# tuannv-github/srsRAN_Project

Hardware: AMD Instinct MI355X
Metric: PDSCH+PUSCH codeblocks/s @ 100 MHz 273-PRB 4x4 MIMO (PDSCH 4 layers, PUSCH 4 layers x 4 rx) (higher is better)
Workload: dtype int8+fp32; 1 GPU; BASELINE metric (PDSCH+PUSCH codeblocks/s @ 100 MHz 273-PRB 4x4 MIMO): full PDSCH+PUSCH slot pipeline, 100 MHz numerology-1 273 PRB, 256QAM R=948/1024; parallelism=single GPU

## Files before the change

### srsran_project_amd/csrc/crc_device.h

```cpp
#pragma once

#include <hip/hip_runtime.h>

#include <cstdint>

namespace srs_amd {

__device__ __forceinline__ uint32_t crc_wave_xor(uint32_t v)
{
#pragma unroll
  for (int o = 32; o >= 1; o >>= 1) {
    v ^= static_cast<uint32_t>(__shfl_xor(static_cast<int>(v), o, 64));
  }
  return v;
}

template <int THREADS>
__device__ __forceinline__ void crc_table8_init(uint32_t* T, uint32_t order, uint32_t polynom)
{
  if (order < 8) {
    return;
  }
  const uint32_t highbit = 1u << order;
  for (uint32_t t = threadIdx.x; t < 256; t += THREADS) {
    uint32_t r = t << (order - 8);
#pragma unroll
    for (int i = 0; i < 8; ++i) {
      r <<= 1;
      if (r & highbit) {
        r ^= polynom;
      }
    }
    T[t] = r;
  }
}

constexpr uint32_t CRC_FETCH_BATCH = 16;
constexpr uint32_t CRC_MAX_ORDER = 24;

template <typename Fetch>
__device__ __forceinline__ uint32_t crc_chunk_contrib(const Fetch&    fetch,
                                                      uint32_t        b0,
                                                      uint32_t        b1,
                                                      uint32_t        n,
                                                      uint32_t        order,
                                                      uint32_t        polynom,
                                                      const uint32_t* table,
                                                      const uint32_t* T,
                                                      uint32_t        to = 0xffffffffu)
{
  to = to == 0xffffffffu ? n : to;
  if (b0 >= b1) {
    return 0;
  }
  const uint32_t highbit = 1u << order;
  const uint32_t mask    = highbit - 1u;
  const uint32_t full    = min(b1, n / 8);
  uint32_t       r       = 0;
  uint32_t       b       = b0;
  if (order >= 8) {
    const uint32_t sh = order - 8;
    for (; b < full; b += CRC_FETCH_BATCH) {
      uint32_t v[CRC_FETCH_BATCH];
#pragma unroll
      for (uint32_t k = 0; k < CRC_FETCH_BATCH; ++k) {
        v[k] = b + k < full ? fetch(b + k) : 0u;
      }
#pragma unroll
      for (uint32_t k = 0; k < CRC_FETCH_BATCH; ++k) {
        if (b + k < full) {
          r = T[r >> sh] ^ ((r << 8) & mask) ^ v[k];
        }
      }
    }
    b = max(b0, full);
  }
  for (; b < b1; ++b) {
    const uint32_t byte = fetch(b);
    const int      nb   = (b * 8 + 8 <= n) ? 8 : static_cast<int>(n - b * 8);
    for (int i = 0; i < nb; ++i) {
      r = (r << 1) | ((byte >> (7 - i)) & 1u);
      if (r & highbit) {
        r ^= polynom;
      }
    }
  }
  const uint32_t  e       = min(n, b1 * 8);
  const uint32_t* tj      = table + (to - e);
  uint32_t        contrib = 0;
#pragma unroll
  for (uint32_t j = 0; j < CRC_MAX_ORDER; ++j) {
    if (j < order) {
      contrib ^= tj[j] & (0u - ((r >> j) & 1u));
    }
  }
  return contrib;
}

__device__ __forceinline__ uint32_t crc_move(uint32_t R, uint32_t d, uint32_t order, const uint32_t* table)
{
  uint32_t out = 0;
#pragma unroll
  for (uint32_t j = 0; j < CRC_MAX_ORDER; ++j) {
    const uint32_t k    = j + d;
    const uint32_t word = k >= order ? table[k - order] : 0u;
    const uint32_t v    = k < order ? (1u << (k & 31u)) : word;
    out ^= (j < order) ? (v & (0u - ((R >> j) & 1u))) : 0u;
  }
  return out;
}

template <typename Fetch>
__device__ __forceinline__ uint32_t crc_chunk_rem(const Fetch& fetch, uint32_t b0, uint32_t b1, uint32_t order,
                                                  const uint32_t* T)
{
  const uint32_t mask = (1u << order) - 1u;
  const uint32_t sh   = order - 8;
  uint32_t       r    = 0;
  for (uint32_t b = b0; b < b1; b += CRC_FETCH_BATCH) {
    uint32_t v[CRC_FETCH_BATCH];
#pragma unroll
    for (uint32_t k = 0; k < CRC_FETCH_BATCH; ++k) {
      v[k] = b + k < b1 ? fetch(b + k) : 0u;
    }
#pragma unroll
    for (uint32_t k = 0; k < CRC_FETCH_BATCH; ++k) {
      if (b + k < b1) {
        r = T[r >> sh] ^ ((r << 8) & mask) ^ v[k];
      }
    }
  }
  return r;
}

__device__ __forceinline__ uint32_t crc_mulmod(uint32_t a, uint32_t c, uint32_t order, uint32_t polynom)
{
  const uint32_t mask = (1u << order) - 1u;
  const uint32_t top  = 1u << (order - 1);
  uint32_t       r    = 0;
#pragma unroll
  for (uint32_t i = 0; i < CRC_MAX_ORDER; ++i) {
    if (i < order) {
      r ^= c & (0u - ((a >> i) & 1u));
      const uint32_t hi = c & top;
      c                 = ((c << 1) & mask) ^ (hi ? (polynom & mask) : 0u);
    }
  }
  return r;
}

__device__ __forceinline__ uint32_t crc_xpow(uint32_t m, uint32_t order, const uint32_t* table)
{
  return m < order ? (1u << m) : table[m - order];
}

template <int THREADS>
__device__ __forceinline__ uint32_t crc_block_xor(uint32_t v, uint32_t* partial)
{
  v = crc_wave_xor(v);
  __syncthreads();
  if ((threadIdx.x & 63) == 0) {
    partial[threadIdx.x >> 6] = v;
  }
  __syncthreads();
  uint32_t crc = 0;
#pragma unroll
  for (int w = 0; w < THREADS / 64; ++w) {
    crc ^= partial[w];
  }
  return crc;
}

template <int THREADS, typename Fetch>
__device__ uint32_t block_crc_bytes(const Fetch&    fetch,
                                    uint32_t        n,
                                    uint32_t        order,
                                    uint32_t        polynom,
                                    const uint32_t* table,
                                    const uint32_t* T,
                                    uint32_t*       partial)
{
  const uint32_t nbytes = (n + 7) / 8;
  const uint32_t per    = (nbytes + THREADS - 1) / THREADS;
  const uint32_t b0     = threadIdx.x * per;
  const uint32_t b1     = min(nbytes, b0 + per);
  return crc_block_xor<THREADS>(crc_chunk_contrib(fetch, b0, b1, n, order, polynom, table, T), partial);
}

__device__ __forceinline__ void attach_crc_bits(uint8_t* row, uint32_t n, uint32_t order, uint32_t crc)
{
  const uint32_t first = n >> 3, last = (n + order - 1) >> 3;
  uint32_t       bytes[4];
#pragma unroll
  for (uint32_t k = 0; k < 4; ++k) {
    bytes[k] = first + k <= last ? row[first + k] : 0u;
  }
#pragma unroll
  for (uint32_t k = 0; k < 4; ++k) {
    if (first + k <= last) {
      uint32_t byte = bytes[k];
#pragma unroll
      for (uint32_t b = 0; b < 8; ++b) {
        const uint32_t pos = 8 * (first + k) + b;
        if (pos >= n && pos < n + order) {
          const uint32_t mask = 0x80u >> b;
          byte                = (byte & ~mask) | (((crc >> (order - 1 - (pos - n))) & 1u) ? mask : 0u);
        }
      }
      row[first + k] = static_cast<uint8_t>(byte);
    }
  }
}

template <int THREADS>
__device__ __forceinline__ void crc_stage_bytes(uint8_t* dst, const uint8_t* row, uint32_t c0, uint32_t n)
{
  const uint8_t* src = row + c0;
  uint32_t       nw  = (reinterpret_cast<uintptr_t>(src) & 3u) == 0 ? n / 4 : 0;
  constexpr int  U   = 8;
  for (uint32_t w0 = threadIdx.x; w0 < nw; w0 += U * THREADS) {
    uint32_t v[U];
#pragma unroll
    for (int r = 0; r < U; ++r) {
      const uint32_t w = w0 + r * THREADS;
      v[r]             = w < nw ? reinterpret_cast<const uint32_t*>(src)[w] : 0u;
    }
#pragma unroll
    for (int r = 0; r < U; ++r) {
      const uint32_t w = w0 + r * THREADS;
      if (w < nw) {
        reinterpret_cast<uint32_t*>(dst)[w] = v[r];
      }
    }
  }
  for (uint32_t i = 4 * nw + threadIdx.x; i < n; i += THREADS) {
    dst[i] = src[i];
  }
}

struct row_fetch {
  const uint8_t* row;
  __device__ uint32_t operator()(uint32_t j) const { return row[j]; }
};

struct lds_chunk_fetch {
  const uint8_t* chunk;
  uint32_t       first;
  __device__ uint32_t operator()(uint32_t j) const { return chunk[j - first]; }
};

}
```

### srsran_project_amd/csrc/ldpc_encode_device.h

```cpp
#pragma once

#include <hip/hip_runtime.h>

#include <cstdint>

namespace srs_amd {

__device__ __forceinline__ uint32_t lds_bits32(const uint32_t* W, uint32_t off)
{
  const uint32_t w = off >> 5;
  return __builtin_amdgcn_alignbit(W[w + 1], W[w], off & 31u);
}

__device__ __forceinline__ uint32_t cyc32(const uint32_t* W, uint32_t cz, uint32_t Z, uint32_t x0, uint32_t s)
{
  uint32_t pos = x0 + s;
  pos -= pos >= Z ? Z : 0u;
  uint32_t v = lds_bits32(W, cz + pos);
  if (pos + 32 > Z) {
    const uint32_t n1 = Z - pos;
    v = (v & ((1u << n1) - 1u)) | (lds_bits32(W, cz) << n1);
  }
  return v;
}

__device__ __forceinline__ void lds_or_bits(uint32_t* W, uint32_t off, uint32_t v, uint32_t n)
{
  v &= n < 32 ? (1u << n) - 1u : 0xffffffffu;
  const uint32_t w = off >> 5, sh = off & 31u;
  atomicOr(&W[w], v << sh);
  if (sh != 0) {
    atomicOr(&W[w + 1], v >> (32 - sh));
  }
}

__host__ __device__ constexpr uint32_t enc_bits_cw_words(uint32_t K, uint32_t M_eff, uint32_t Z)
{
  return ((K + M_eff) * Z + 31) / 32 + 2;
}
__host__ __device__ constexpr uint32_t enc_bits_lds_words(uint32_t K, uint32_t M_eff, uint32_t Z)
{
  return enc_bits_cw_words(K, M_eff, Z) + 4 * ((Z + 31) / 32) + (Z + 31) / 32 + 2;
}

template <int NT>
__device__ __forceinline__ void encode_bits_parity(uint32_t*       cw,
                                                   uint32_t*       lam,
                                                   uint32_t*       ls,
                                                   const uint32_t* edges,
                                                   const int32_t*  row_start,
                                                   int             bg,
                                                   uint32_t        K,
                                                   uint32_t        Z,
                                                   uint32_t        M_eff,
                                                   int32_t         p0_shift,
                                                   const int32_t (&core_a)[3],
                                                   uint32_t        j)
{
  const uint32_t kz = K * Z;
  const uint32_t nq = (Z + 31) / 32;
  for (uint32_t task = j; task < 4 * nq; task += NT) {
    const uint32_t r = task / nq, x0 = 32 * (task - r * nq);
    uint32_t       acc = 0;
    for (int e = row_start[r]; e < row_start[r + 1]; ++e) {
      const uint32_t ed   = edges[e];
      const uint32_t base = ed & 0xffffu;
      if (base >= kz) {
        break;
      }
      acc ^= cyc32(cw, base, Z, x0, ed >> 16);
    }
    lam[task] = acc;
  }
  __syncthreads();
  for (uint32_t q = j; q < nq; q += NT) {
    const uint32_t n = min(32u, Z - 32 * q);
    const uint32_t v = lam[q] ^ lam[nq + q] ^ lam[2 * nq + q] ^ lam[3 * nq + q];
    ls[q]            = n < 32 ? v & ((1u << n) - 1u) : v;
  }
  __syncthreads();

  const uint32_t sh0 = (Z - static_cast<uint32_t>(p0_shift) % Z) % Z;
  for (uint32_t q = j; q < nq; q += NT) {
    lds_or_bits(cw, kz + 32 * q, cyc32(ls, 0, Z, 32 * q, sh0), min(32u, Z - 32 * q));
  }
  __syncthreads();

  for (uint32_t q = j; q < nq; q += NT) {
    const uint32_t x0 = 32 * q, n = min(32u, Z - x0);
    auto           at = [&](int s) { return cyc32(cw, kz, Z, x0, static_cast<uint32_t>(s)); };
    uint32_t       p1, p2, p3;
    p1 = lam[q] ^ at(core_a[0]);
    if (bg == 1) {
      p2 = lam[nq + q] ^ at(core_a[1]) ^ p1;
      p3 = lam[2 * nq + q] ^ p2;
    } else {
      p2 = lam[nq + q] ^ p1;
      p3 = lam[2 * nq + q] ^ at(core_a[2]) ^ p2;
    }
    lds_or_bits(cw, kz + Z + x0, p1, n);
    lds_or_bits(cw, kz + 2 * Z + x0, p2, n);
    lds_or_bits(cw, kz + 3 * Z + x0, p3, n);
  }
  __syncthreads();

  const uint32_t hz = kz + 4 * Z;
  for (uint32_t task = j; task < (M_eff - 4) * nq; task += NT) {
    const uint32_t rr = task / nq, r = 4 + rr, x0 = 32 * (task - rr * nq);
    uint32_t       acc = 0;
    for (int e = row_start[r]; e < row_start[r + 1]; ++e) {
      const uint32_t ed   = edges[e];
      const uint32_t base = ed & 0xffffu;
      if (base >= hz) {
        break;
      }
      acc ^= cyc32(cw, base, Z, x0, ed >> 16);
    }
    lds_or_bits(cw, (K + r) * Z + x0, acc, min(32u, Z - x0));
  }
  __syncthreads();
}

}
```

### srsran_project_amd/csrc/pdsch_encoder.hip

```cpp
#include <hip/hip_runtime.h>

#include <algorithm>
#include <atomic>
#include <cstdlib>

#include "crc_device.h"
#include "ldpc_codec_args.h"
#include "ldpc_common.h"
#include "ldpc_encode_device.h"
#include "rate_match_device.h"
#include "sch_args.h"

namespace srs_amd {
namespace {

constexpr uint32_t PE_CW_BYTES  = 66 * MAX_LIFTING_SIZE / 8;
constexpr uint32_t PE_ENC_WORDS = enc_bits_lds_words(22, 46, MAX_LIFTING_SIZE);

__device__ __forceinline__ uint32_t pe_out_byte(const uint8_t* s_cw, const rm_geometry& g, const fast_div& divL,
                                                uint32_t off, uint32_t E, uint32_t Kq, uint32_t b)
{
  uint32_t byte = 0;
#pragma unroll
  for (uint32_t k = 0; k < 8; ++k) {
    const uint32_t gbit = 8 * b + k;
    if (gbit < off || gbit >= off + E) {
      continue;
    }
    const uint32_t o = gbit - off;
    uint32_t       i, j;
    if (g.Qm == 6) {
      i = __umulhi(o >> 1, 0xAAAAAAABu) >> 1;
      j = o - 6 * i;
    } else {
      const uint32_t sh = g.Qm == 8 ? 3 : g.Qm == 4 ? 2 : g.Qm == 2 ? 1 : 0;
      i                 = o >> sh;
      j                 = o & (g.Qm - 1);
    }
    uint32_t w = g.rank0 + j * Kq + i;
    if (w >= g.L) {
      w -= g.L;
      if (w >= g.L) {
        divL.div(w, w);
      }
    }
    const uint32_t p = w < g.nof_info ? w : w + g.F;
    byte |= ((s_cw[p >> 3] >> (7 - (p & 7))) & 1u) << (7 - k);
  }
  return byte;
}

struct pe_lds {
  uint32_t T24b[256];
  uint32_t Ttb[256];
  uint32_t lw[PE_ENC_WORDS];
  uint32_t edges[MAX_EDGES];
  __attribute__((aligned(16))) uint8_t s_cw[PE_CW_BYTES + 8];
  uint32_t partial[4];
};

template <int NT>
__device__ __forceinline__ uint32_t pe_xor(uint32_t v, uint32_t* partial)
{
  if constexpr (NT == 64) {
    return crc_wave_xor(v);
  } else {
    return crc_block_xor<NT>(v, partial);
  }
}

template <int NT>
__device__ __forceinline__ void pe_message(const pdsch_fused_args& a, const tb_desc& d, uint32_t r, uint32_t n_data,
                                           uint32_t kz, uint8_t* s_cw, uint32_t j)
{
  const uint8_t* tb  = a.tbs + d.tb_offset;
  const uint32_t ob  = r * d.cb_info_bits;
  const uint32_t nmb = (kz + 7) / 8;
  if ((ob & 7u) == 0) {
    const uintptr_t base  = reinterpret_cast<uintptr_t>(tb) + ob / 8;
    const uint32_t  nfull = n_data / 32;
    for (uint32_t q = j; q < nfull; q += NT) {
      const uintptr_t  addr = base + 4 * q;
      const uint32_t*  p4   = reinterpret_cast<const uint32_t*>(addr & ~uintptr_t(3));
      const uint32_t   sh   = static_cast<uint32_t>(addr & 3u);
      const uint32_t   lo   = p4[0];
      const uint32_t   hi   = sh != 0 ? p4[1] : 0u;
      reinterpret_cast<uint32_t*>(s_cw)[q] = sh != 0 ? __builtin_amdgcn_alignbyte(hi, lo, sh) : lo;
    }
    for (uint32_t q = nfull + j; q < (nmb + 3) / 4; q += NT) {
      uint32_t w = 0;
      for (uint32_t b = 0; b < 4; ++b) {
        const uint32_t jb = 4 * q + b;
        uint32_t       v  = 0;
        for (uint32_t k = 0; k < 8 && 8 * jb + k < n_data; ++k) {
          const uint32_t p = ob + 8 * jb + k;
          v |= ((tb[p >> 3] >> (7 - (p & 7))) & 1u) << (7 - k);
        }
        w |= v << (8 * b);
      }
      reinterpret_cast<uint32_t*>(s_cw)[q] = w;
    }
    return;
  }
  for (uint32_t q = j; q < (nmb + 3) / 4; q += NT) {
    uint32_t w = 0;
#pragma unroll
    for (uint32_t b = 0; b < 4; ++b) {
      const uint32_t jb = 4 * q + b;
      uint32_t       v  = 0;
      if (8 * jb + 8 <= n_data) {
        const uint32_t p  = ob + 8 * jb;
        const uint32_t sh = p & 7u;
        uint32_t       x  = static_cast<uint32_t>(tb[p >> 3]) << 8;
        if (sh != 0) {
          x |= tb[(p >> 3) + 1];
        }
        v = (x >> (8 - sh)) & 0xffu;
      } else if (8 * jb < n_data) {
        for (uint32_t k = 0; k < 8 && 8 * jb + k < n_data; ++k) {
          const uint32_t p = ob + 8 * jb + k;
          v |= ((tb[p >> 3] >> (7 - (p & 7))) & 1u) << (7 - k);
        }
      }
      w |= v << (8 * b);
    }
    reinterpret_cast<uint32_t*>(s_cw)[q] = w;
  }
}

__device__ __forceinline__ void pe_crc24_pair(const uint8_t* s_cw, uint32_t b0, uint32_t b1, uint32_t n,
                                              uint32_t polyA, const uint32_t* tableA, const uint32_t* TA,
                                              uint32_t polyB, const uint32_t* tableB, const uint32_t* TB,
                                              uint32_t& outA, uint32_t& outB)
{
  outA = 0;
  outB = 0;
  if (b0 >= b1) {
    return;
  }
  constexpr uint32_t highbit = 1u << 24, mask = highbit - 1u;
  const uint32_t     full    = min(b1, n / 8);
  uint32_t           rA = 0, rB = 0;
  for (uint32_t b = b0; b < full; b += CRC_FETCH_BATCH) {
    uint32_t v[CRC_FETCH_BATCH];
#pragma unroll
    for (uint32_t k = 0; k < CRC_FETCH_BATCH; ++k) {
      v[k] = b + k < full ? s_cw[b + k] : 0u;
    }
#pragma unroll
    for (uint32_t k = 0; k < CRC_FETCH_BATCH; ++k) {
      if (b + k < full) {
        rA = TA[rA >> 16] ^ ((rA << 8) & mask) ^ v[k];
        rB = TB[rB >> 16] ^ ((rB << 8) & mask) ^ v[k];
      }
    }
  }
  for (uint32_t b = max(b0, full); b < b1; ++b) {
    const uint32_t byte = s_cw[b];
    const int      nb   = (b * 8 + 8 <= n) ? 8 : static_cast<int>(n - b * 8);
    for (int i = 0; i < nb; ++i) {
      const uint32_t bit = (byte >> (7 - i)) & 1u;
      rA                 = (rA << 1) | bit;
      rB                 = (rB << 1) | bit;
      rA ^= (rA & highbit) ? polyA : 0u;
      rB ^= (rB & highbit) ? polyB : 0u;
    }
  }
  const uint32_t  e  = min(n, b1 * 8);
  const uint32_t* ta = tableA + (n - e);
  const uint32_t* tb = tableB + (n - e);
#pragma unroll
  for (uint32_t j = 0; j < 24; ++j) {
    outA ^= ta[j] & (0u - ((rA >> j) & 1u));
    outB ^= tb[j] & (0u - ((rB >> j) & 1u));
  }
}

template <int NT>
__device__ __forceinline__ void pe_finish(const pdsch_fused_args& a, pe_lds& s, uint32_t cb, uint32_t t,
                                          const tb_desc& d, uint32_t j, uint32_t& staged_off, uint32_t& staged_ne)
{
  const rm_geometry  g   = a.geos[a.row_geo[cb]];
  const enc_row_desc er  = a.enc_rows[cb];
  const uint32_t     E   = a.row_E[cb];
  const uint32_t     off = a.row_out[cb];
  const uint32_t     Z   = er.Z;
  const uint32_t     Kb  = g.nof_sys / Z + 2;
  const int          bg  = Kb == 22 ? 1 : 2;
  const uint32_t     kz  = Kb * Z;
  uint8_t*           s_cw = s.s_cw;
  if (d.nof_segments > 1) {
    const uint32_t cbi = d.cb_info_bits;
    const uint32_t nb  = (cbi + 7) / 8;
    const uint32_t per = (nb + NT - 1) / NT;
    const uint32_t b0  = j * per;
    const uint32_t r   = cb - d.row0;
    uint32_t       crc;
    if (r + 1 < d.nof_segments) {
      uint32_t tb_part;
      pe_crc24_pair(s_cw, b0, min(nb, b0 + per), cbi, a.crc24b_poly, a.crc24b_table, s.T24b, a.crc24a_poly,
                    a.crc24a_table, s.Ttb, crc, tb_part);
      crc     = pe_xor<NT>(crc, s.partial);
      tb_part = pe_xor<NT>(tb_part, s.partial);
      if (j == 0) {
        a.tb_parts[static_cast<size_t>(t) * a.part_stride + r] = tb_part;
      }
    } else {
      crc = pe_xor<NT>(crc_chunk_contrib(lds_chunk_fetch{s_cw, 0}, b0, min(nb, b0 + per), cbi, 24, a.crc24b_poly,
                                         a.crc24b_table, s.T24b),
                       s.partial);
    }
    if (j == 0) {
      attach_crc_bits(s_cw, cbi, 24, crc);
    }
    __syncthreads();
  }
  const uint32_t nq  = (Z + 31) / 32;
  const uint32_t ncw = enc_bits_cw_words(Kb, er.M_eff, Z);
  uint32_t*      cwb = s.lw;
  uint32_t*      lam = s.lw + ncw;
  uint32_t*      ls  = lam + 4 * nq;
  const uint32_t nmw = (kz + 31) / 32;
  for (uint32_t w = j; w < ncw; w += NT) {
    uint32_t v = 0;
    if (w < nmw) {
      v = __builtin_bitreverse32(__builtin_bswap32(reinterpret_cast<const uint32_t*>(s_cw)[w]));
      if (32 * w + 32 > kz) {
        v &= (1u << (kz - 32 * w)) - 1u;
      }
    }
    cwb[w] = v;
  }
  for (uint32_t w = j; w < nq + 2; w += NT) {
    ls[w] = 0;
  }
  const uint32_t* ge = a.edges + er.edge_off;
  const uint32_t  ne = static_cast<uint32_t>(a.row_start[bg - 1][er.M_eff]);
  if (er.edge_off != staged_off || ne != staged_ne) {
    for (uint32_t e = j; e < ne; e += NT) {
      s.edges[e] = ge[e];
    }
    staged_off = er.edge_off;
    staged_ne  = ne;
  }
  __syncthreads();
  const int32_t core_a[3] = {static_cast<int32_t>(er.core_a[0]), static_cast<int32_t>(er.core_a[1]),
                             static_cast<int32_t>(er.core_a[2])};
  encode_bits_parity<NT>(cwb, lam, ls, s.edges, a.row_start[bg - 1], bg, Kb, Z, er.M_eff,
                                 static_cast<int32_t>(er.p0_shift), core_a, j);
  const uint32_t nbits = er.pack_bits;
  for (uint32_t m = j; m < (nbits + 31) / 32; m += NT) {
    uint32_t v = lds_bits32(cwb, 2 * Z + 32 * m);
    if (32 * m + 32 > nbits) {
      v &= (1u << (nbits - 32 * m)) - 1u;
    }
    reinterpret_cast<uint32_t*>(s_cw)[m] = __builtin_bswap32(__builtin_bitreverse32(v));
  }
  __syncthreads();
  const fast_div divL(g.L);
  const uint32_t Kq    = E / g.Qm;
  const uint32_t first = (off + 7) / 8;
  const uint32_t whole = (off + E) / 8;
  const uint32_t G        = ((off & 7u) == 0 && g.Qm >= 2) ? Kq / 8 : 0;
  const uint32_t fast_end = first + G * g.Qm;
  for (uint32_t gi = j; gi < G; gi += NT) {
    uint64_t x = 0;
#pragma unroll
    for (uint32_t jj = 0; jj < 8; ++jj) {
      if (jj < g.Qm) {
        uint32_t w = g.rank0 + jj * Kq + 8 * gi;
        if (w >= g.L) {
          w -= g.L;
          if (w >= g.L) {
            divL.div(w, w);
          }
        }
        x |= static_cast<uint64_t>(rm_walk_byte(s_cw, g, w)) << (56 - 8 * jj);
      }
    }
    x            = transpose8x8(x);
    uint64_t acc = 0;
#pragma unroll
    for (uint32_t q = 0; q < 8; ++q) {
      acc = (acc << g.Qm) | ((x >> (64 - 8 * q - g.Qm)) & ((1u << g.Qm) - 1u));
    }
    uint8_t* o = a.cw + first + gi * g.Qm;
    for (uint32_t q = 0; q < g.Qm; ++q) {
      o[q] = static_cast<uint8_t>(acc >> (8 * (g.Qm - 1 - q)));
    }
  }
  for (uint32_t b = fast_end + j; b < whole; b += NT) {
    a.cw[b] = static_cast<uint8_t>(pe_out_byte(s_cw, g, divL, off, E, Kq, b));
  }
  if (j < 2) {
    const bool     last_seg = cb == d.row0 + d.nof_segments - 1;
    const uint32_t b        = j == 0 ? off / 8 : whole;
    const bool partial =
        j == 0 ? (off & 7u) != 0 : ((off + E) & 7u) != 0 && (whole != off / 8 || (off & 7u) == 0);
    if (partial) {
      uint32_t mask = 0;
      for (uint32_t k = 0; k < 8; ++k) {
        const uint32_t gbit = 8 * b + k;
        mask |= (gbit >= off && (gbit < off + E || last_seg)) ? (0x80u >> k) : 0u;
      }
      const uint32_t v  = pe_out_byte(s_cw, g, divL, off, E, Kq, b);
      uint32_t*      w4 = reinterpret_cast<uint32_t*>(a.cw + (b & ~3u));
      const uint32_t sh = 8 * (b & 3u);
      atomicAnd(w4, ~(mask << sh));
      atomicOr(w4, v << sh);
    }
  }
  __syncthreads();
}

template <int NT>
__global__ __launch_bounds__(NT) void pdsch_cb_kernel(pdsch_fused_args a)
{
  __shared__ pe_lds s;
  crc_table8_init<NT>(s.T24b, 24, a.crc24b_poly);
  crc_table8_init<NT>(s.Ttb, 24, a.crc24a_poly);
  uint32_t       tb_table_order = 24;
  uint32_t       staged_off = 0, staged_ne = 0;
  const uint32_t j              = threadIdx.x;

  const uint32_t n = a.last_only == 1 ? a.nof_tbs : a.nof_cbs;
  for (uint32_t k = blockIdx.x; k < n; k += gridDim.x) {
    const uint32_t cb   = a.last_only == 1 ? a.last_rows[k] : k;
    const uint32_t t    = a.row_tb[cb];
    const tb_desc  d    = a.tds[t];
    const uint32_t r    = cb - d.row0;
    const uint32_t C    = d.nof_segments;
    const bool     last = r == C - 1;
    if ((a.last_only == 0) == last) {
      continue;
    }
    const uint32_t L    = d.tb_crc_bits;
    const uint32_t n_data = last ? d.cb_info_bits - L - d.zero_pad : d.cb_info_bits;
    const uint32_t kz     = (a.geos[a.row_geo[cb]].nof_sys / a.enc_rows[cb].Z + 2) * a.enc_rows[cb].Z;
    uint32_t tb_crc = 0;
    if (last) {
      if (tb_table_order != L) {
        crc_table8_init<NT>(s.Ttb, L, L == 16 ? a.crc16_poly : a.crc24a_poly);
        tb_table_order = L;
      }
      for (uint32_t i = j; i + 1 < C; i += NT) {
        tb_crc ^= crc_move(a.tb_parts[static_cast<size_t>(t) * a.part_stride + i],
                           d.tbs_bits - (i + 1) * d.cb_info_bits, 24, a.crc24a_table);
      }
    }
    pe_message<NT>(a, d, r, n_data, kz, s.s_cw, j);
    __syncthreads();
    if (last) {
      const uint32_t nb  = (n_data + 7) / 8;
      const uint32_t per = (nb + NT - 1) / NT;
      const uint32_t b0  = j * per;
      tb_crc ^= crc_chunk_contrib(lds_chunk_fetch{s.s_cw, 0}, b0, min(nb, b0 + per), n_data, L,
                                  L == 16 ? a.crc16_poly : a.crc24a_poly, L == 16 ? a.crc16_table : a.crc24a_table,
                                  s.Ttb);
      tb_crc = pe_xor<NT>(tb_crc, s.partial);
      if (j == 0) {
        attach_crc_bits(s.s_cw, n_data, L, tb_crc);
      }
      __syncthreads();
    }
    pe_finish<NT>(a, s, cb, t, d, j, staged_off, staged_ne);
  }
}

constexpr int PE_MAX_DEVICES = 64;

template <int NT>
uint32_t pe_resident_workgroups()
{
  static std::atomic<uint32_t> known[PE_MAX_DEVICES] = {};
  int                          dev = 0, per_cu = 0, cus = 0;
  if (hipGetDevice(&dev) != hipSuccess || dev < 0 || dev >= PE_MAX_DEVICES) {
    (void)hipGetLastError();
    return 65535u;
  }
  uint32_t n = known[dev].load(std::memory_order_relaxed);
  if (n == 0) {
    if (hipDeviceGetAttribute(&cus, hipDeviceAttributeMultiprocessorCount, dev) != hipSuccess || cus <= 0 ||
        hipOccupancyMaxActiveBlocksPerMultiprocessor(&per_cu, pdsch_cb_kernel<NT>, NT, 0) != hipSuccess ||
        per_cu <= 0) {
      (void)hipGetLastError();
      return 65535u;
    }
    n = static_cast<uint32_t>(per_cu) * static_cast<uint32_t>(cus);
    known[dev].store(n, std::memory_order_relaxed);
  }
  return n;
}

}

hipError_t launch_pdsch_fused(const pdsch_fused_args& a, hipStream_t stream)
{
  if (a.nof_cbs == 0) {
    return hipSuccess;
  }
  const char* wg       = std::getenv("SRSRAN_AMD_PDSCH_WG");
  const char* tail     = std::getenv("SRSRAN_AMD_PDSCH_TAIL_WG");
  const bool  big      = wg != nullptr && wg[0] == '2';
  const bool  big_tail = tail == nullptr || tail[0] == '2';
  const char*    gs  = std::getenv("SRSRAN_AMD_PDSCH_GRID");
  const uint32_t cap = gs != nullptr && std::atoi(gs) > 0 ? static_cast<uint32_t>(std::atoi(gs))
                       : big                              ? pe_resident_workgroups<256>()
                                                          : pe_resident_workgroups<64>();
  auto cb_launch = [&](uint32_t last_only, uint32_t n, bool wide) {
    pdsch_fused_args x = a;
    x.last_only        = last_only;
    const dim3 grid(std::min(n, last_only == 0 ? std::min(cap, 65535u) : 65535u));
    if (wide) {
      hipLaunchKernelGGL(pdsch_cb_kernel<256>, grid, dim3(256), 0, stream, x);
    } else {
      hipLaunchKernelGGL(pdsch_cb_kernel<64>, grid, dim3(64), 0, stream, x);
    }
  };
  if (a.nof_cbs > a.nof_tbs) {
    cb_launch(0, a.nof_cbs, big);
  }
  cb_launch(1, a.nof_tbs, big_tail);
  return hipGetLastError();
}

}
```

Measured before the change: 25.14 million codeblocks/s.

## Prefetch next codeblock metadata and message, vectorize CRC, group rate matching

The PDSCH fused kernel is restructured so each workgroup prefetches the next codeblock's descriptors and message words into registers while it is still encoding the current one, which hides global-load latency behind compute. It also adds several other changes: word-wide CRC over LDS with an optional single-polynomial path, mask-based CRC bit attachment, staging of row_start and systematic edge counts in LDS for a batched parity loop, and QM-templated grouped rate matching that processes 32-bit groups. An optional timing probe is added behind a compile flag. The cost is higher register pressure from the prefetch state, which could lower occupancy, plus a larger LDS footprint that is guarded by an assert.

```diff
diff --git a/srsran_project_amd/csrc/crc_device.h b/srsran_project_amd/csrc/crc_device.h
--- a/srsran_project_amd/csrc/crc_device.h
+++ b/srsran_project_amd/csrc/crc_device.h
@@ -190,6 +190,9 @@
 __device__ __forceinline__ void attach_crc_bits(uint8_t* row, uint32_t n, uint32_t order, uint32_t crc)
 {
   const uint32_t first = n >> 3, last = (n + order - 1) >> 3;
+  const uint32_t sh    = 32 - (n & 7u) - order;
+  const uint32_t mask  = ((1u << order) - 1u) << sh;
+  const uint32_t field = (crc << sh) & mask;
   uint32_t       bytes[4];
 #pragma unroll
   for (uint32_t k = 0; k < 4; ++k) {
@@ -198,16 +201,8 @@
 #pragma unroll
   for (uint32_t k = 0; k < 4; ++k) {
     if (first + k <= last) {
-      uint32_t byte = bytes[k];
-#pragma unroll
-      for (uint32_t b = 0; b < 8; ++b) {
-        const uint32_t pos = 8 * (first + k) + b;
-        if (pos >= n && pos < n + order) {
-          const uint32_t mask = 0x80u >> b;
-          byte                = (byte & ~mask) | (((crc >> (order - 1 - (pos - n))) & 1u) ? mask : 0u);
-        }
-      }
-      row[first + k] = static_cast<uint8_t>(byte);
+      const uint32_t m = (mask >> (24 - 8 * k)) & 0xffu;
+      row[first + k]   = static_cast<uint8_t>((bytes[k] & ~m) | ((field >> (24 - 8 * k)) & 0xffu));
     }
   }
 }
diff --git a/srsran_project_amd/csrc/ldpc_encode_device.h b/srsran_project_amd/csrc/ldpc_encode_device.h
--- a/srsran_project_amd/csrc/ldpc_encode_device.h
+++ b/srsran_project_amd/csrc/ldpc_encode_device.h
@@ -43,32 +43,55 @@
   return enc_bits_cw_words(K, M_eff, Z) + 4 * ((Z + 31) / 32) + (Z + 31) / 32 + 2;
 }
 
-template <int NT>
+#ifndef ENC_STAMP
+#define ENC_STAMP(i)                                                                                                 \
+  do {                                                                                                               \
+  } while (0)
+#endif
+
+template <int NT, typename RS>
 __device__ __forceinline__ void encode_bits_parity(uint32_t*       cw,
                                                    uint32_t*       lam,
                                                    uint32_t*       ls,
                                                    const uint32_t* edges,
-                                                   const int32_t*  row_start,
+                                                   const RS*       row_start,
                                                    int             bg,
                                                    uint32_t        K,
                                                    uint32_t        Z,
                                                    uint32_t        M_eff,
                                                    int32_t         p0_shift,
                                                    const int32_t (&core_a)[3],
-                                                   uint32_t        j)
+                                                   uint32_t        j,
+                                                   const uint16_t* nsys = nullptr)
 {
   const uint32_t kz = K * Z;
   const uint32_t nq = (Z + 31) / 32;
   for (uint32_t task = j; task < 4 * nq; task += NT) {
     const uint32_t r = task / nq, x0 = 32 * (task - r * nq);
     uint32_t       acc = 0;
-    for (int e = row_start[r]; e < row_start[r + 1]; ++e) {
-      const uint32_t ed   = edges[e];
-      const uint32_t base = ed & 0xffffu;
-      if (base >= kz) {
-        break;
+    if (nsys != nullptr) {
+      const uint32_t e0 = static_cast<uint32_t>(row_start[r]), e1 = e0 + nsys[r];
+      for (uint32_t e = e0; e < e1; e += 4) {
+        uint32_t ed[4];
+#pragma unroll
+        for (uint32_t k = 0; k < 4; ++k) {
+          ed[k] = edges[min(e + k, e1 - 1)];
+        }
+#pragma unroll
+        for (uint32_t k = 0; k < 4; ++k) {
+          const uint32_t v = cyc32(cw, ed[k] & 0xffffu, Z, x0, ed[k] >> 16);
+          acc ^= e + k < e1 ? v : 0u;
+        }
       }
-      acc ^= cyc32(cw, base, Z, x0, ed >> 16);
+    } else {
+      for (int e = row_start[r]; e < row_start[r + 1]; ++e) {
+        const uint32_t ed   = edges[e];
+        const uint32_t base = ed & 0xffffu;
+        if (base >= kz) {
+          break;
+        }
+        acc ^= cyc32(cw, base, Z, x0, ed >> 16);
+      }
     }
     lam[task] = acc;
   }
@@ -79,12 +102,14 @@
     ls[q]            = n < 32 ? v & ((1u << n) - 1u) : v;
   }
   __syncthreads();
+  ENC_STAMP(7);
 
   const uint32_t sh0 = (Z - static_cast<uint32_t>(p0_shift) % Z) % Z;
   for (uint32_t q = j; q < nq; q += NT) {
     lds_or_bits(cw, kz + 32 * q, cyc32(ls, 0, Z, 32 * q, sh0), min(32u, Z - 32 * q));
   }
   __syncthreads();
+  ENC_STAMP(8);
 
   for (uint32_t q = j; q < nq; q += NT) {
     const uint32_t x0 = 32 * q, n = min(32u, Z - x0);
diff --git a/srsran_project_amd/csrc/pdsch_encoder.hip b/srsran_project_amd/csrc/pdsch_encoder.hip
--- a/srsran_project_amd/csrc/pdsch_encoder.hip
+++ b/srsran_project_amd/csrc/pdsch_encoder.hip
@@ -3,6 +3,24 @@
 #include <algorithm>
 #include <atomic>
 #include <cstdlib>
+
+#ifdef SRS_AMD_PDSCH_PROBE
+constexpr uint32_t PE_PROBE_WG = 4096;
+__device__ uint64_t g_pdsch_probe[2][PE_PROBE_WG][2][16];
+__shared__ uint32_t pe_probe_launch, pe_probe_visit;
+#define PE_STAMP(i)                                                                                                  \
+  do {                                                                                                               \
+    if (threadIdx.x == 0 && blockIdx.x < PE_PROBE_WG && pe_probe_visit < 2) {                                        \
+      g_pdsch_probe[pe_probe_launch][blockIdx.x][pe_probe_visit][i] =                                                \
+          (i) == 0 || (i) == 15 ? __builtin_amdgcn_s_memrealtime() : __builtin_amdgcn_s_memtime();                   \
+    }                                                                                                                \
+  } while (0)
+#define ENC_STAMP(i) PE_STAMP(i)
+#else
+#define PE_STAMP(i)                                                                                                  \
+  do {                                                                                                               \
+  } while (0)
+#endif
 
 #include "crc_device.h"
 #include "ldpc_codec_args.h"
@@ -57,7 +75,10 @@
   uint32_t edges[MAX_EDGES];
   __attribute__((aligned(16))) uint8_t s_cw[PE_CW_BYTES + 8];
   uint32_t partial[4];
+  uint16_t rs[48];
+  uint16_t nsys[4];
 };
+static_assert(sizeof(pe_lds) <= 10240, "pe_lds: fewer workgroups per CU");
 
 template <int NT>
 __device__ __forceinline__ uint32_t pe_xor(uint32_t v, uint32_t* partial)
@@ -69,23 +90,113 @@
   }
 }
 
+struct pe_cb {
+  uint32_t     k;
+  bool         valid;
+  bool         last;
+  bool         skip;
+  uint32_t     cb, t, gi, E, off;
+  uint32_t     r, n_data, Kb, kz;
+  enc_row_desc er;
+  tb_desc      d;
+  rm_geometry  g;
+};
+
+__device__ __forceinline__ void pe_level0(const pdsch_fused_args& a, uint32_t n, uint32_t k, pe_cb& c)
+{
+  c.k     = k;
+  c.valid = k < n;
+  c.cb    = 0;
+  if (c.valid) {
+    c.cb = a.last_only == 1 ? a.last_rows[k] : k;
+  }
+}
+
+__device__ __forceinline__ void pe_level1(const pdsch_fused_args& a, pe_cb& c)
+{
+  c.t = c.gi = c.E = c.off = 0;
+  c.er                     = enc_row_desc{};
+  if (c.valid) {
+    c.t   = a.row_tb[c.cb];
+    c.gi  = a.row_geo[c.cb];
+    c.er  = a.enc_rows[c.cb];
+    c.E   = a.row_E[c.cb];
+    c.off = a.row_out[c.cb];
+  }
+}
+
+__device__ __forceinline__ void pe_level2(const pdsch_fused_args& a, pe_cb& c)
+{
+  c.d    = tb_desc{};
+  c.g    = rm_geometry{};
+  c.last = c.skip = false;
+  c.r = c.n_data = c.Kb = c.kz = 0;
+  if (c.valid) {
+    c.d    = a.tds[c.t];
+    c.g    = a.geos[c.gi];
+    c.r    = c.cb - c.d.row0;
+    c.last = c.r == c.d.nof_segments - 1;
+    c.skip = (a.last_only == 0) == c.last;
+    c.n_data = c.last ? c.d.cb_info_bits - c.d.tb_crc_bits - c.d.zero_pad : c.d.cb_info_bits;
+    const uint32_t Z = c.er.Z;
+    c.Kb             = c.g.nof_sys == 20 * Z ? 22 : c.g.nof_sys == 8 * Z ? 10 : c.g.nof_sys / Z + 2;
+    c.kz             = c.Kb * Z;
+  }
+}
+
 template <int NT>
-__device__ __forceinline__ void pe_message(const pdsch_fused_args& a, const tb_desc& d, uint32_t r, uint32_t n_data,
-                                           uint32_t kz, uint8_t* s_cw, uint32_t j)
-{
-  const uint8_t* tb  = a.tbs + d.tb_offset;
-  const uint32_t ob  = r * d.cb_info_bits;
-  const uint32_t nmb = (kz + 7) / 8;
+struct pe_msg {
+  static constexpr uint32_t U = NT == 64 ? 5 : 2;
+  static_assert(22 * MAX_LIFTING_SIZE / 32 <= U * NT, "pe_msg: rounds");
+  uint32_t lo[U], hi[U];
+};
+
+template <int NT>
+__device__ __forceinline__ void pe_msg_load(const pdsch_fused_args& a, const pe_cb& c, uint32_t j, pe_msg<NT>& m)
+{
+#pragma unroll
+  for (uint32_t k = 0; k < pe_msg<NT>::U; ++k) {
+    m.lo[k] = 0;
+    m.hi[k] = 0;
+  }
+  const uint32_t ob = c.r * c.d.cb_info_bits;
+  if (!c.valid || c.skip || (ob & 7u) != 0) {
+    return;
+  }
+  const uintptr_t base  = reinterpret_cast<uintptr_t>(a.tbs + c.d.tb_offset) + ob / 8;
+  const uint32_t* p4    = reinterpret_cast<const uint32_t*>(base & ~uintptr_t(3));
+  const uint32_t  sh    = static_cast<uint32_t>(base & 3u);
+  const uint32_t  nfull = c.n_data / 32;
+#pragma unroll
+  for (uint32_t k = 0; k < pe_msg<NT>::U; ++k) {
+    const uint32_t q = j + k * NT;
+    if (q < nfull) {
+      m.lo[k] = p4[q];
+      if (sh != 0) {
+        m.hi[k] = p4[q + 1];
+      }
+    }
+  }
+}
+
+template <int NT>
+__device__ __forceinline__ void pe_msg_store(const pdsch_fused_args& a, const pe_cb& c, const pe_msg<NT>& m,
+                                             uint8_t* s_cw, uint32_t j)
+{
+  const tb_desc& d      = c.d;
+  const uint32_t n_data = c.n_data;
+  const uint8_t* tb     = a.tbs + d.tb_offset;
+  const uint32_t ob     = c.r * d.cb_info_bits;
+  const uint32_t nmb    = (c.kz + 7) / 8;
   if ((ob & 7u) == 0) {
-    const uintptr_t base  = reinterpret_cast<uintptr_t>(tb) + ob / 8;
-    const uint32_t  nfull = n_data / 32;
-    for (uint32_t q = j; q < nfull; q += NT) {
-      const uintptr_t  addr = base + 4 * q;
-      const uint32_t*  p4   = reinterpret_cast<const uint32_t*>(addr & ~uintptr_t(3));
-      const uint32_t   sh   = static_cast<uint32_t>(addr & 3u);
-      const uint32_t   lo   = p4[0];
-      const uint32_t   hi   = sh != 0 ? p4[1] : 0u;
-      reinterpret_cast<uint32_t*>(s_cw)[q] = sh != 0 ? __builtin_amdgcn_alignbyte(hi, lo, sh) : lo;
+    const uint32_t sh    = static_cast<uint32_t>((reinterpret_cast<uintptr_t>(tb) + ob / 8) & 3u);
+    const uint32_t nfull = n_data / 32;
+#pragma unroll
+    for (uint32_t k = 0; k < pe_msg<NT>::U; ++k) {
+      const uint32_t q = j + k * NT;
+      if (q < nfull) {
+        reinterpret_cast<uint32_t*>(s_cw)[q] = __builtin_amdgcn_alignbyte(m.hi[k], m.lo[k], sh);
+      }
     }
     for (uint32_t q = nfull + j; q < (nmb + 3) / 4; q += NT) {
       uint32_t w = 0;
@@ -128,42 +239,68 @@
   }
 }
 
-__device__ __forceinline__ void pe_crc24_pair(const uint8_t* s_cw, uint32_t b0, uint32_t b1, uint32_t n,
-                                              uint32_t polyA, const uint32_t* tableA, const uint32_t* TA,
-                                              uint32_t polyB, const uint32_t* tableB, const uint32_t* TB,
-                                              uint32_t& outA, uint32_t& outB)
+template <int NT>
+__device__ __forceinline__ uint32_t pe_crc_slice(uint32_t nb)
+{
+  return ((nb + NT - 1) / NT + 3u) & ~3u;
+}
+
+template <bool PAIR>
+__device__ __forceinline__ void pe_crc_lds(const uint8_t* s_cw, uint32_t b0, uint32_t b1, uint32_t n, uint32_t orderA,
+                                           uint32_t polyA, const uint32_t* tableA, const uint32_t* TA, uint32_t polyB,
+                                           const uint32_t* tableB, const uint32_t* TB, uint32_t& outA, uint32_t& outB)
 {
   outA = 0;
   outB = 0;
   if (b0 >= b1) {
     return;
   }
-  constexpr uint32_t highbit = 1u << 24, mask = highbit - 1u;
-  const uint32_t     full    = min(b1, n / 8);
+  constexpr uint32_t highB = 1u << 24, maskB = highB - 1u;
+  const uint32_t     highA = 1u << orderA, maskA = highA - 1u, shA = orderA - 8;
+  const uint32_t     full  = min(b1, n / 8);
+  const uint32_t*    w4    = reinterpret_cast<const uint32_t*>(s_cw);
   uint32_t           rA = 0, rB = 0;
-  for (uint32_t b = b0; b < full; b += CRC_FETCH_BATCH) {
-    uint32_t v[CRC_FETCH_BATCH];
-#pragma unroll
-    for (uint32_t k = 0; k < CRC_FETCH_BATCH; ++k) {
-      v[k] = b + k < full ? s_cw[b + k] : 0u;
-    }
-#pragma unroll
-    for (uint32_t k = 0; k < CRC_FETCH_BATCH; ++k) {
-      if (b + k < full) {
-        rA = TA[rA >> 16] ^ ((rA << 8) & mask) ^ v[k];
-        rB = TB[rB >> 16] ^ ((rB << 8) & mask) ^ v[k];
-      }
-    }
-  }
-  for (uint32_t b = max(b0, full); b < b1; ++b) {
+  auto               step = [&](uint32_t byte) {
+    rA = TA[rA >> shA] ^ ((rA << 8) & maskA) ^ byte;
+    if constexpr (PAIR) {
+      rB = TB[rB >> 16] ^ ((rB << 8) & maskB) ^ byte;
+    }
+  };
+  auto word = [&](uint32_t w) {
+    step(w & 0xffu);
+    step((w >> 8) & 0xffu);
+    step((w >> 16) & 0xffu);
+    step(w >> 24);
+  };
+  uint32_t b = b0;
+  for (; b + 16 <= full; b += 16) {
+    uint32_t v[4];
+#pragma unroll
+    for (uint32_t k = 0; k < 4; ++k) {
+      v[k] = w4[b / 4 + k];
+    }
+#pragma unroll
+    for (uint32_t k = 0; k < 4; ++k) {
+      word(v[k]);
+    }
+  }
+  for (; b + 4 <= full; b += 4) {
+    word(w4[b / 4]);
+  }
+  for (; b < full; ++b) {
+    step(s_cw[b]);
+  }
+  for (; b < b1; ++b) {
     const uint32_t byte = s_cw[b];
     const int      nb   = (b * 8 + 8 <= n) ? 8 : static_cast<int>(n - b * 8);
     for (int i = 0; i < nb; ++i) {
       const uint32_t bit = (byte >> (7 - i)) & 1u;
       rA                 = (rA << 1) | bit;
-      rB                 = (rB << 1) | bit;
-      rA ^= (rA & highbit) ? polyA : 0u;
-      rB ^= (rB & highbit) ? polyB : 0u;
+      rA ^= (rA & highA) ? polyA : 0u;
+      if constexpr (PAIR) {
+        rB = (rB << 1) | bit;
+        rB ^= (rB & highB) ? polyB : 0u;
+      }
     }
   }
   const uint32_t  e  = min(n, b1 * 8);
@@ -171,50 +308,150 @@
   const uint32_t* tb = tableB + (n - e);
 #pragma unroll
   for (uint32_t j = 0; j < 24; ++j) {
-    outA ^= ta[j] & (0u - ((rA >> j) & 1u));
-    outB ^= tb[j] & (0u - ((rB >> j) & 1u));
+    if (j < orderA) {
+      outA ^= ta[j] & (0u - ((rA >> j) & 1u));
+    }
+    if constexpr (PAIR) {
+      outB ^= tb[j] & (0u - ((rB >> j) & 1u));
+    }
+  }
+}
+
+__device__ __forceinline__ uint32_t pe_walk32(const uint32_t* W, uint32_t base, const rm_geometry& g, uint32_t w)
+{
+  const uint32_t B = w < g.nof_info ? g.nof_info : g.L;
+  uint32_t       v = lds_bits32(W, base + (w < g.nof_info ? w : w + g.F));
+  if (w + 32 > B) {
+    const uint32_t n1 = B - w;
+    const uint32_t w1 = B == g.L ? 0u : B;
+    const uint32_t B1 = w1 < g.nof_info ? g.nof_info : g.L;
+    if (w1 + (32 - n1) <= B1) {
+      const uint32_t v1 = lds_bits32(W, base + (w1 < g.nof_info ? w1 : w1 + g.F));
+      v                 = (v & ((1u << n1) - 1u)) | (v1 << n1);
+    } else {
+      v = 0;
+#pragma unroll 1
+      for (uint32_t k = 0; k < 32; ++k) {
+        uint32_t ww = w + k;
+        while (ww >= g.L) {
+          ww -= g.L;
+        }
+        const uint32_t p = base + (ww < g.nof_info ? ww : ww + g.F);
+        v |= ((W[p >> 5] >> (p & 31u)) & 1u) << k;
+      }
+    }
+  }
+  return v;
+}
+
+template <uint32_t QM, int NT>
+__device__ __forceinline__ void pe_rm_groups(const uint32_t* W, uint32_t base, const rm_geometry& g,
+                                             const fast_div& divL, uint32_t Kq, uint32_t G, uint32_t rem_bytes,
+                                             uint8_t* o, uint32_t j)
+{
+  const uint32_t NG  = G + (rem_bytes != 0 ? 1u : 0u);
+  const uint32_t oal = static_cast<uint32_t>(reinterpret_cast<uintptr_t>(o) & 3u);
+  for (uint32_t t = j; 4 * t < NG; t += NT) {
+    uint32_t v[QM];
+#pragma unroll
+    for (uint32_t jj = 0; jj < QM; ++jj) {
+      uint32_t w = g.rank0 + jj * Kq + 32 * t;
+      if (w >= g.L) {
+        w -= g.L;
+        if (w >= g.L) {
+          divL.div(w, w);
+        }
+      }
+      v[jj] = pe_walk32(W, base, g, w);
+    }
+#pragma unroll
+    for (uint32_t q = 0; q < 4; ++q) {
+      const uint32_t gi = 4 * t + q;
+      if (gi < NG) {
+        uint64_t x = 0;
+#pragma unroll
+        for (uint32_t jj = 0; jj < QM; ++jj) {
+          x |= static_cast<uint64_t>((v[jj] >> (8 * q)) & 0xffu) << (56 - 8 * jj);
+        }
+        x = transpose8x8(x);
+        uint64_t out = x;
+        if constexpr (QM != 8) {
+          uint64_t acc = 0;
+#pragma unroll
+          for (uint32_t k = 0; k < 8; ++k) {
+            acc = (acc << QM) | ((x >> (8 * k + 8 - QM)) & ((1u << QM) - 1u));
+          }
+          out = __builtin_bswap64(acc << (64 - 8 * QM));
+        }
+        uint8_t* og = o + gi * QM;
+        if (gi >= G) {
+          for (uint32_t k = 0; k < rem_bytes; ++k) {
+            og[k] = static_cast<uint8_t>(out >> (8 * k));
+          }
+        } else if ((QM == 8 || QM == 4) && oal == 0) {
+          reinterpret_cast<uint32_t*>(og)[0] = static_cast<uint32_t>(out);
+          if constexpr (QM == 8) {
+            reinterpret_cast<uint32_t*>(og)[1] = static_cast<uint32_t>(out >> 32);
+          }
+        } else if ((oal & 1u) == 0) {
+#pragma unroll
+          for (uint32_t k = 0; k < QM; k += 2) {
+            *reinterpret_cast<uint16_t*>(og + k) = static_cast<uint16_t>(out >> (8 * k));
+          }
+        } else {
+#pragma unroll
+          for (uint32_t k = 0; k < QM; ++k) {
+            og[k] = static_cast<uint8_t>(out >> (8 * k));
+          }
+        }
+      }
+    }
   }
 }
 
 template <int NT>
-__device__ __forceinline__ void pe_finish(const pdsch_fused_args& a, pe_lds& s, uint32_t cb, uint32_t t,
-                                          const tb_desc& d, uint32_t j, uint32_t& staged_off, uint32_t& staged_ne)
-{
-  const rm_geometry  g   = a.geos[a.row_geo[cb]];
-  const enc_row_desc er  = a.enc_rows[cb];
-  const uint32_t     E   = a.row_E[cb];
-  const uint32_t     off = a.row_out[cb];
-  const uint32_t     Z   = er.Z;
-  const uint32_t     Kb  = g.nof_sys / Z + 2;
-  const int          bg  = Kb == 22 ? 1 : 2;
-  const uint32_t     kz  = Kb * Z;
-  uint8_t*           s_cw = s.s_cw;
+__device__ __forceinline__ void pe_finish(const pdsch_fused_args& a, pe_lds& s, const pe_cb& c, pe_cb& nx,
+                                          pe_msg<NT>& m, uint32_t j, uint32_t& staged_off, uint32_t& staged_ne)
+{
+  const rm_geometry&  g    = c.g;
+  const enc_row_desc& er   = c.er;
+  const tb_desc&      d    = c.d;
+  const uint32_t      E    = c.E;
+  const uint32_t      off  = c.off;
+  const uint32_t      Z    = er.Z;
+  const uint32_t      Kb   = c.Kb;
+  const int           bg   = Kb == 22 ? 1 : 2;
+  const uint32_t      kz   = c.kz;
+  uint8_t*            s_cw = s.s_cw;
   if (d.nof_segments > 1) {
     const uint32_t cbi = d.cb_info_bits;
     const uint32_t nb  = (cbi + 7) / 8;
-    const uint32_t per = (nb + NT - 1) / NT;
+    const uint32_t per = pe_crc_slice<NT>(nb);
     const uint32_t b0  = j * per;
-    const uint32_t r   = cb - d.row0;
-    uint32_t       crc;
-    if (r + 1 < d.nof_segments) {
-      uint32_t tb_part;
-      pe_crc24_pair(s_cw, b0, min(nb, b0 + per), cbi, a.crc24b_poly, a.crc24b_table, s.T24b, a.crc24a_poly,
-                    a.crc24a_table, s.Ttb, crc, tb_part);
+    uint32_t       crc, tb_part;
+    if (!c.last) {
+      pe_crc_lds<true>(s_cw, b0, min(nb, b0 + per), cbi, 24, a.crc24a_poly, a.crc24a_table, s.Ttb, a.crc24b_poly,
+                       a.crc24b_table, s.T24b, tb_part, crc);
       crc     = pe_xor<NT>(crc, s.partial);
       tb_part = pe_xor<NT>(tb_part, s.partial);
       if (j == 0) {
-        a.tb_parts[static_cast<size_t>(t) * a.part_stride + r] = tb_part;
+        a.tb_parts[static_cast<size_t>(c.t) * a.part_stride + c.r] = tb_part;
       }
     } else {
-      crc = pe_xor<NT>(crc_chunk_contrib(lds_chunk_fetch{s_cw, 0}, b0, min(nb, b0 + per), cbi, 24, a.crc24b_poly,
-                                         a.crc24b_table, s.T24b),
-                       s.partial);
-    }
+      pe_crc_lds<false>(s_cw, b0, min(nb, b0 + per), cbi, 24, a.crc24b_poly, a.crc24b_table, s.T24b, 0,
+                        a.crc24b_table, s.T24b, crc, tb_part);
+      crc = pe_xor<NT>(crc, s.partial);
+    }
+    PE_STAMP(4);
     if (j == 0) {
       attach_crc_bits(s_cw, cbi, 24, crc);
     }
     __syncthreads();
-  }
+  } else {
+    PE_STAMP(4);
+  }
+  PE_STAMP(5);
+  pe_level1(a, nx);
   const uint32_t nq  = (Z + 31) / 32;
   const uint32_t ncw = enc_bits_cw_words(Kb, er.M_eff, Z);
   uint32_t*      cwb = s.lw;
@@ -240,60 +477,72 @@
     for (uint32_t e = j; e < ne; e += NT) {
       s.edges[e] = ge[e];
     }
+    for (uint32_t i = j; i <= er.M_eff; i += NT) {
+      s.rs[i] = static_cast<uint16_t>(a.row_start[bg - 1][i]);
+    }
+    __syncthreads();
+    if (j < 4) {
+      uint32_t cnt = 0;
+      for (uint32_t e = s.rs[j]; e < s.rs[j + 1] && (s.edges[e] & 0xffffu) < kz; ++e) {
+        ++cnt;
+      }
+      s.nsys[j] = static_cast<uint16_t>(cnt);
+    }
     staged_off = er.edge_off;
     staged_ne  = ne;
   }
   __syncthreads();
+  PE_STAMP(6);
   const int32_t core_a[3] = {static_cast<int32_t>(er.core_a[0]), static_cast<int32_t>(er.core_a[1]),
                              static_cast<int32_t>(er.core_a[2])};
-  encode_bits_parity<NT>(cwb, lam, ls, s.edges, a.row_start[bg - 1], bg, Kb, Z, er.M_eff,
-                                 static_cast<int32_t>(er.p0_shift), core_a, j);
+  encode_bits_parity<NT>(cwb, lam, ls, s.edges, s.rs, bg, Kb, Z, er.M_eff, static_cast<int32_t>(er.p0_shift), core_a,
+                         j, s.nsys);
+  PE_STAMP(9);
+  pe_level2(a, nx);
   const uint32_t nbits = er.pack_bits;
-  for (uint32_t m = j; m < (nbits + 31) / 32; m += NT) {
-    uint32_t v = lds_bits32(cwb, 2 * Z + 32 * m);
-    if (32 * m + 32 > nbits) {
-      v &= (1u << (nbits - 32 * m)) - 1u;
-    }
-    reinterpret_cast<uint32_t*>(s_cw)[m] = __builtin_bswap32(__builtin_bitreverse32(v));
+  for (uint32_t mw = j; mw < (nbits + 31) / 32; mw += NT) {
+    uint32_t v = lds_bits32(cwb, 2 * Z + 32 * mw);
+    if (32 * mw + 32 > nbits) {
+      v &= (1u << (nbits - 32 * mw)) - 1u;
+    }
+    reinterpret_cast<uint32_t*>(s_cw)[mw] = __builtin_bswap32(__builtin_bitreverse32(v));
   }
   __syncthreads();
+  PE_STAMP(10);
+  pe_msg_load<NT>(a, nx, j, m);
   const fast_div divL(g.L);
   const uint32_t Kq    = E / g.Qm;
   const uint32_t first = (off + 7) / 8;
   const uint32_t whole = (off + E) / 8;
-  const uint32_t G        = ((off & 7u) == 0 && g.Qm >= 2) ? Kq / 8 : 0;
-  const uint32_t fast_end = first + G * g.Qm;
-  for (uint32_t gi = j; gi < G; gi += NT) {
-    uint64_t x = 0;
-#pragma unroll
-    for (uint32_t jj = 0; jj < 8; ++jj) {
-      if (jj < g.Qm) {
-        uint32_t w = g.rank0 + jj * Kq + 8 * gi;
-        if (w >= g.L) {
-          w -= g.L;
-          if (w >= g.L) {
-            divL.div(w, w);
-          }
-        }
-        x |= static_cast<uint64_t>(rm_walk_byte(s_cw, g, w)) << (56 - 8 * jj);
-      }
-    }
-    x            = transpose8x8(x);
-    uint64_t acc = 0;
-#pragma unroll
-    for (uint32_t q = 0; q < 8; ++q) {
-      acc = (acc << g.Qm) | ((x >> (64 - 8 * q - g.Qm)) & ((1u << g.Qm) - 1u));
-    }
-    uint8_t* o = a.cw + first + gi * g.Qm;
-    for (uint32_t q = 0; q < g.Qm; ++q) {
-      o[q] = static_cast<uint8_t>(acc >> (8 * (g.Qm - 1 - q)));
-    }
-  }
+  const bool     grouped   = (off & 7u) == 0 && (g.Qm == 2 || g.Qm == 4 || g.Qm == 6 || g.Qm == 8);
+  const uint32_t G         = grouped ? Kq / 8 : 0;
+  const uint32_t rem_bytes = grouped ? ((Kq & 7u) * g.Qm) / 8 : 0;
+  const uint32_t fast_end  = first + G * g.Qm + rem_bytes;
+  if (grouped) {
+    uint8_t* const  obase = a.cw + first;
+    const uint32_t* cb0   = cwb;
+    switch (g.Qm) {
+      case 2:
+        pe_rm_groups<2, NT>(cb0, 2 * Z, g, divL, Kq, G, rem_bytes, obase, j);
+        break;
+      case 4:
+        pe_rm_groups<4, NT>(cb0, 2 * Z, g, divL, Kq, G, rem_bytes, obase, j);
+        break;
+      case 6:
+        pe_rm_groups<6, NT>(cb0, 2 * Z, g, divL, Kq, G, rem_bytes, obase, j);
+        break;
+      default:
+        pe_rm_groups<8, NT>(cb0, 2 * Z, g, divL, Kq, G, rem_bytes, obase, j);
+        break;
+    }
+  }
+  PE_STAMP(11);
   for (uint32_t b = fast_end + j; b < whole; b += NT) {
     a.cw[b] = static_cast<uint8_t>(pe_out_byte(s_cw, g, divL, off, E, Kq, b));
   }
+  PE_STAMP(12);
   if (j < 2) {
-    const bool     last_seg = cb == d.row0 + d.nof_segments - 1;
+    const bool     last_seg = c.last;
     const uint32_t b        = j == 0 ? off / 8 : whole;
     const bool partial =
         j == 0 ? (off & 7u) != 0 : ((off + E) & 7u) != 0 && (whole != off / 8 || (off & 7u) == 0);
@@ -311,6 +560,7 @@
     }
   }
   __syncthreads();
+  PE_STAMP(13);
 }
 
 template <int NT>
@@ -322,48 +572,77 @@
   uint32_t       tb_table_order = 24;
   uint32_t       staged_off = 0, staged_ne = 0;
   const uint32_t j              = threadIdx.x;
+#ifdef SRS_AMD_PDSCH_PROBE
+  if (j == 0) {
+    pe_probe_launch = a.last_only;
+    pe_probe_visit  = 0;
+  }
+#endif
 
   const uint32_t n = a.last_only == 1 ? a.nof_tbs : a.nof_cbs;
-  for (uint32_t k = blockIdx.x; k < n; k += gridDim.x) {
-    const uint32_t cb   = a.last_only == 1 ? a.last_rows[k] : k;
-    const uint32_t t    = a.row_tb[cb];
-    const tb_desc  d    = a.tds[t];
-    const uint32_t r    = cb - d.row0;
-    const uint32_t C    = d.nof_segments;
-    const bool     last = r == C - 1;
-    if ((a.last_only == 0) == last) {
-      continue;
-    }
-    const uint32_t L    = d.tb_crc_bits;
-    const uint32_t n_data = last ? d.cb_info_bits - L - d.zero_pad : d.cb_info_bits;
-    const uint32_t kz     = (a.geos[a.row_geo[cb]].nof_sys / a.enc_rows[cb].Z + 2) * a.enc_rows[cb].Z;
+  pe_cb      c;
+  pe_msg<NT> m;
+  PE_STAMP(0);
+  PE_STAMP(1);
+  pe_level0(a, n, blockIdx.x, c);
+  pe_level1(a, c);
+  pe_level2(a, c);
+  pe_msg_load<NT>(a, c, j, m);
+  for (;;) {
+    while (c.valid && c.skip) {
+      pe_level0(a, n, c.k + gridDim.x, c);
+      pe_level1(a, c);
+      pe_level2(a, c);
+      pe_msg_load<NT>(a, c, j, m);
+    }
+    if (!c.valid) {
+      break;
+    }
+    const tb_desc& d = c.d;
+    const uint32_t C = d.nof_segments;
+    const uint32_t L = d.tb_crc_bits;
     uint32_t tb_crc = 0;
-    if (last) {
+    if (c.last) {
       if (tb_table_order != L) {
         crc_table8_init<NT>(s.Ttb, L, L == 16 ? a.crc16_poly : a.crc24a_poly);
         tb_table_order = L;
       }
       for (uint32_t i = j; i + 1 < C; i += NT) {
-        tb_crc ^= crc_move(a.tb_parts[static_cast<size_t>(t) * a.part_stride + i],
+        tb_crc ^= crc_move(a.tb_parts[static_cast<size_t>(c.t) * a.part_stride + i],
                            d.tbs_bits - (i + 1) * d.cb_info_bits, 24, a.crc24a_table);
       }
     }
-    pe_message<NT>(a, d, r, n_data, kz, s.s_cw, j);
+    PE_STAMP(2);
+    pe_msg_store<NT>(a, c, m, s.s_cw, j);
     __syncthreads();
-    if (last) {
-      const uint32_t nb  = (n_data + 7) / 8;
-      const uint32_t per = (nb + NT - 1) / NT;
+    PE_STAMP(3);
+    pe_cb nx;
+    pe_level0(a, n, c.k + gridDim.x, nx);
+    if (c.last) {
+      const uint32_t nb  = (c.n_data + 7) / 8;
+      const uint32_t per = pe_crc_slice<NT>(nb);
       const uint32_t b0  = j * per;
-      tb_crc ^= crc_chunk_contrib(lds_chunk_fetch{s.s_cw, 0}, b0, min(nb, b0 + per), n_data, L,
-                                  L == 16 ? a.crc16_poly : a.crc24a_poly, L == 16 ? a.crc16_table : a.crc24a_table,
-                                  s.Ttb);
-      tb_crc = pe_xor<NT>(tb_crc, s.partial);
+      uint32_t       own, unused;
+      pe_crc_lds<false>(s.s_cw, b0, min(nb, b0 + per), c.n_data, L, L == 16 ? a.crc16_poly : a.crc24a_poly,
+                        L == 16 ? a.crc16_table : a.crc24a_table, s.Ttb, 0, a.crc24a_table, s.Ttb, own, unused);
+      tb_crc = pe_xor<NT>(tb_crc ^ own, s.partial);
       if (j == 0) {
-        attach_crc_bits(s.s_cw, n_data, L, tb_crc);
+        attach_crc_bits(s.s_cw, c.n_data, L, tb_crc);
       }
       __syncthreads();
     }
-    pe_finish<NT>(a, s, cb, t, d, j, staged_off, staged_ne);
+    pe_finish<NT>(a, s, c, nx, m, j, staged_off, staged_ne);
+#ifdef SRS_AMD_PDSCH_PROBE
+    PE_STAMP(15);
+    if (j == 0) {
+      pe_probe_visit += 1;
+    }
+    if (nx.valid) {
+      PE_STAMP(0);
+      PE_STAMP(1);
+    }
+#endif
+    c = nx;
   }
 }
 
@@ -393,6 +672,25 @@
 }
 
 }
+
+#ifdef SRS_AMD_PDSCH_PROBE
+extern "C" int srs_amd_pdsch_probe_read(void* host, uint64_t bytes, int clear)
+{
+  if (bytes > sizeof(g_pdsch_probe)) {
+    bytes = sizeof(g_pdsch_probe);
+  }
+  if (hipMemcpyFromSymbol(host, HIP_SYMBOL(g_pdsch_probe), bytes) != hipSuccess) {
+    return -2;
+  }
+  if (clear) {
+    static const uint64_t zero[2 * PE_PROBE_WG * 2 * 16] = {};
+    if (hipMemcpyToSymbol(HIP_SYMBOL(g_pdsch_probe), zero, sizeof(zero)) != hipSuccess) {
+      return -2;
+    }
+  }
+  return 0;
+}
+#endif
 
 hipError_t launch_pdsch_fused(const pdsch_fused_args& a, hipStream_t stream)
 {
```

Result: no change. 25.02 million codeblocks/s (-0.5%).
